# tdhock/PeakSegDisk

Hardware: AMD Instinct MI355X
Metric: coverage bins/sec across 64-penalty grid (higher is better)
Workload: dtype f64; 1 GPU; 1000000-bin synthetic Poisson coverage x 64-penalty grid per GPU (BASELINE.json configs[1]); bins=1000000, penalties=64, penalty_grid=10^seq(-1,5), 15 significant digits, seed=1+rank

## Files before the change

include/peaksegdisk_hip.h:

```cpp
#ifndef PEAKSEGDISK_HIP_H
#define PEAKSEGDISK_HIP_H

#include <stddef.h>

#ifdef __cplusplus
extern "C" {
#endif

#define ERROR_PENALTY_NOT_FINITE 1
#define ERROR_PENALTY_NEGATIVE 2
#define ERROR_UNABLE_TO_OPEN_BEDGRAPH 3
#define ERROR_NOT_ENOUGH_COLUMNS 4
#define ERROR_NON_INTEGER_DATA 5
#define ERROR_INCONSISTENT_CHROMSTART_CHROMEND 6
#define ERROR_WRITING_COST_FUNCTIONS 7
#define ERROR_WRITING_LOSS_OUTPUT 8
#define ERROR_NO_DATA 9
#define ERROR_PENALTY_NOT_NUMERIC 10
#define ERROR_WRITING_SEGMENTS_OUTPUT 11
#define ERROR_NO_HIP_DEVICE 12
#define ERROR_DEVICE_SOLVER 13
#define ERROR_DEVICE_MEMORY 14
#define ERROR_SEARCH_ARGUMENTS 15
#define ERROR_SEARCH_TOO_MANY_PEAKS 16
// ... 236 lines not shown
                                               const long long *contig_n_bases,
                                               const int *const *contig_counts, int counts_on_device,
                                               int n_penalties, const double *penalties,
                                               unsigned long long arena_pieces, int folds,
                                               unsigned long long seed, psd_problem_set **out);
int peakseg_hip_problem_set_create_reads_folds(
    int device, int n_contigs, const long long *n_reads, const int *const *read_start,
    const int *const *read_end, const int *const *read_count, int reads_on_device,
    const int *extent_start, const int *extent_end, int bases_counted, int n_penalties,
    const double *penalties, unsigned long long arena_pieces, int folds, unsigned long long seed,
    psd_problem_set **out);
int peakseg_hip_fold_max_count(void);
int peakseg_hip_fold_units_last_ms(float *ms);

int peakseg_hip_penalty_fit(int device, int n, int p, const double *x_std, const double *lo,
                            const double *hi, const int *fold, int n_folds, int n_reg,
                            const double *reg, double gram_lambda_max, double threshold,
                            int max_iterations, double *weights_out, int *iterations_out,
                            double *criterion_out, int *converged_out, long long *incorrect_out,
                            double *hinge_out);
int peakseg_hip_penalty_fit_last_ms(float *ms);
int peakseg_hip_penalty_fit_max_features(void);

int peakseg_hip_search_place_penalties(double under_penalty, double over_penalty, double secant,
                                       int extras, double *out);

int peakseg_hip_problem_set_loss(psd_problem_set *set, int problem, double *out);

long long peakseg_hip_problem_set_cycles(psd_problem_set *set, int problem);
void peakseg_hip_measured_rates(double *lat_rate, double *thr_rate);

long long peakseg_hip_spin_limit(void);
int peakseg_hip_problem_set_max_spin(psd_problem_set *set, int problem);

int peakseg_hip_problem_set_set_penalty(psd_problem_set *set, int problem, double penalty);

void peakseg_hip_problem_set_destroy(psd_problem_set *set);

int peakseg_hip_parse_probe(const char *path, int use_fast, int *n_lines,
                            unsigned long long *hash);

int peakseg_hip_dense_encode_probe(int device, int n_contigs, const long long *n_bases,
                                   const int *const *counts, int counts_on_device,
                                   long long *runs_out, int *count_out, int *weight_out,
                                   int *run_end_out, int *min_out, int *max_out,
                                   long long *sum_out);
int peakseg_hip_dense_tile_bases(void);
int peakseg_hip_dense_last_encode_ms(float *count_ms, float *scan_ms, float *scatter_ms);

int peakseg_hip_reads_pileup_probe(int device, int n_contigs, const long long *n_reads,
                                   const int *const *read_start, const int *const *read_end,
                                   const int *const *read_count, int reads_on_device,
                                   const int *extent_start, const int *extent_end, int bases_counted,
                                   int *coverage_out, long long *runs_out, int *count_out,
                                   int *weight_out, int *run_end_out);
int peakseg_hip_reads_last_pileup_ms(float *scatter_ms, float *scan_ms);

long long peakseg_hip_peak_clusters_probe(int device, int n_members, const long long *n_peaks,
                                          const int *const *peak_start, const int *const *peak_end,
                                          int *clusterStart_out, int *clusterEnd_out, int *peaks_out,
                                          int *samples_out, int *m_peaks_out);

int peakseg_hip_paste_double(double x, char *buf, size_t buf_len);

int peakseg_hip_problem_set_profile(psd_problem_set *set, int problem, long long *out);

// ... 10 lines not shown
```

peaksegdisk_amd/_native.py:

```python
import ctypes
import os

_HERE = os.path.dirname(os.path.abspath(__file__))
LIB_PATH = os.path.join(_HERE, "lib", "libpeaksegdisk_hip.so")

ERROR_NO_HIP_DEVICE = 12
ERROR_DEVICE_SOLVER = 13
ERROR_DEVICE_MEMORY = 14
ERROR_DENSE_ARGUMENTS = 17
ERROR_READS_ARGUMENTS = 18
ERROR_LABEL_ARGUMENTS = 19
ERROR_FEATURE_ARGUMENTS = 20
ERROR_FIT_ARGUMENTS = 21
ERROR_REGION_ARGUMENTS = 22
ERROR_HELDOUT_ARGUMENTS = 23


class PsdResult(ctypes.Structure):
    _fields_ = [
        ("status", ctypes.c_int),
        ("kernel_status", ctypes.c_int),
        ("n_segments", ctypes.c_int),
        ("n_peaks", ctypes.c_int),
        ("n_equality_constraints", ctypes.c_int),
# ... 93 lines not shown
    lib.PeakSegFPOP_parallel_search_batch.argtypes = [
        c.c_int, c.POINTER(c.c_char_p), c.POINTER(c.c_int), c.c_int, c.c_int, c.c_int,
        c.POINTER(PsdSearchRow), c.POINTER(c.c_int), c.POINTER(c.c_int), c.POINTER(c.c_int)]
    lib.PeakSegFPOP_parallel_search_batch.restype = c.c_int
    lib.peakseg_hip_problem_set_set_penalty.argtypes = [c.c_void_p, c.c_int, c.c_double]
    lib.peakseg_hip_problem_set_set_penalty.restype = c.c_int
    lib.peakseg_hip_problem_set_arena_bytes_used.argtypes = [c.c_void_p]
    lib.peakseg_hip_problem_set_arena_bytes_used.restype = c.c_ulonglong
    lib.peakseg_hip_problem_set_checkpoint_interval.argtypes = [c.c_void_p]
    lib.peakseg_hip_problem_set_checkpoint_interval.restype = c.c_int
    lib.peakseg_hip_paste_double.argtypes = [c.c_double, c.c_char_p, c.c_size_t]
    lib.peakseg_hip_paste_double.restype = c.c_int
    lib.peakseg_hip_problem_set_solve_stats.argtypes = [
        c.c_void_p, c.POINTER(c.c_int), c.POINTER(c.c_ulonglong)]
    lib.peakseg_hip_problem_set_solve_stats.restype = c.c_int
    lib.peakseg_hip_device_clock_khz.argtypes = [c.c_int]
    lib.peakseg_hip_device_clock_khz.restype = c.c_int
    lib.peakseg_hip_problem_set_park_stats.argtypes = [
        c.c_void_p, c.POINTER(c.c_int), c.POINTER(c.c_ulonglong)]
    lib.peakseg_hip_problem_set_park_stats.restype = c.c_int
    lib.peakseg_hip_problem_set_pack_tables.argtypes = [
        c.c_void_p, c.c_void_p, c.POINTER(c.c_void_p), c.POINTER(c.c_void_p)]
    lib.peakseg_hip_problem_set_pack_tables.restype = c.c_longlong
    lib.peakseg_hip_problem_set_packed_download.argtypes = [c.c_void_p, c.c_void_p, c.c_void_p]
    lib.peakseg_hip_problem_set_packed_download.restype = c.c_int
    lib.peakseg_hip_problem_set_cycles.argtypes = [c.c_void_p, c.c_int]
    lib.peakseg_hip_problem_set_cycles.restype = c.c_longlong
    lib.peakseg_hip_measured_rates.argtypes = [c.POINTER(c.c_double), c.POINTER(c.c_double)]
    lib.peakseg_hip_measured_rates.restype = None
    lib.peakseg_hip_spin_limit.argtypes = []
    lib.peakseg_hip_spin_limit.restype = c.c_longlong
    lib.peakseg_hip_problem_set_max_spin.argtypes = [c.c_void_p, c.c_int]
    lib.peakseg_hip_problem_set_max_spin.restype = c.c_int
    lib.peakseg_hip_last_warning.argtypes = []
    lib.peakseg_hip_last_warning.restype = c.c_char_p
    lib.peakseg_hip_problem_set_arena_stats.argtypes = [
        c.c_void_p, c.POINTER(c.c_ulonglong), c.POINTER(c.c_int), c.POINTER(c.c_int)]
    lib.peakseg_hip_problem_set_arena_stats.restype = c.c_int
    lib.peakseg_hip_last_fanout.argtypes = [
        c.c_int, c.POINTER(c.c_int), c.POINTER(c.c_int), c.POINTER(c.c_double)]
    lib.peakseg_hip_last_fanout.restype = c.c_int
    lib.peakseg_hip_last_fanout_entries.argtypes = [c.c_int, c.POINTER(c.c_int)]
    lib.peakseg_hip_last_fanout_entries.restype = c.c_int
    lib.peakseg_hip_problem_set_create_dense.argtypes = [
        c.c_int, c.c_int, c.POINTER(c.c_longlong), c.POINTER(c.c_void_p), c.c_int,
        c.c_int, c.POINTER(c.c_int), c.POINTER(c.c_double), c.c_ulonglong,
        c.POINTER(c.c_void_p)]
    lib.peakseg_hip_problem_set_create_dense.restype = c.c_int
    lib.peakseg_hip_problem_set_pack_segments.argtypes = [
        c.c_void_p, c.c_void_p, c.c_void_p, c.POINTER(c.c_void_p), c.POINTER(c.c_void_p),
        c.POINTER(c.c_void_p)]
    lib.peakseg_hip_problem_set_pack_segments.restype = c.c_longlong
    lib.peakseg_hip_problem_set_packed_segments_download.argtypes = [
        c.c_void_p, c.c_void_p, c.c_void_p, c.c_void_p]
    lib.peakseg_hip_problem_set_packed_segments_download.restype = c.c_int
    lib.peakseg_hip_problem_set_loss.argtypes = [c.c_void_p, c.c_int, c.POINTER(c.c_double)]
    lib.peakseg_hip_problem_set_loss.restype = c.c_int
    lib.peakseg_hip_dense_encode_probe.argtypes = [
        c.c_int, c.c_int, c.POINTER(c.c_longlong), c.POINTER(c.c_void_p), c.c_int,
        c.c_void_p, c.c_void_p, c.c_void_p, c.c_void_p, c.c_void_p, c.c_void_p, c.c_void_p]
    lib.peakseg_hip_dense_encode_probe.restype = c.c_int
    lib.peakseg_hip_dense_tile_bases.argtypes = []
    lib.peakseg_hip_dense_tile_bases.restype = c.c_int
    lib.peakseg_hip_dense_last_encode_ms.argtypes = [
        c.POINTER(c.c_float), c.POINTER(c.c_float), c.POINTER(c.c_float)]
    lib.peakseg_hip_dense_last_encode_ms.restype = c.c_int
# ... 117 lines not shown
        c.POINTER(c.c_double), c.c_ulonglong, c.c_int, c.c_ulonglong, c.POINTER(c.c_void_p)]
    lib.peakseg_hip_problem_set_create_dense_folds.restype = c.c_int
    lib.peakseg_hip_problem_set_create_reads_folds.argtypes = reads + [
        c.c_int, c.POINTER(c.c_double), c.c_ulonglong, c.c_int, c.c_ulonglong, c.POINTER(c.c_void_p)]
    lib.peakseg_hip_problem_set_create_reads_folds.restype = c.c_int
    lib.peakseg_hip_fold_max_count.argtypes = []
    lib.peakseg_hip_fold_max_count.restype = c.c_int
    lib.peakseg_hip_fold_units_last_ms.argtypes = [c.POINTER(c.c_float)]
    lib.peakseg_hip_fold_units_last_ms.restype = c.c_int
    lib.peakseg_hip_search_place_penalties.argtypes = [
        c.c_double, c.c_double, c.c_double, c.c_int, c.POINTER(c.c_double)]
    lib.peakseg_hip_search_place_penalties.restype = c.c_int
    return lib


EXPORTED_SYMBOLS = [
    "PeakSegFPOP_disk", "PeakSegFPOP_disk_batch", "PeakSegFPOP_status_message",
    "peakseg_hip_set_print", "peakseg_hip_device_count", "peakseg_hip_last_error",
    "peakseg_hip_problem_set_create", "peakseg_hip_problem_set_solve",
    "peakseg_hip_problem_set_result", "peakseg_hip_problem_set_segments",
    "peakseg_hip_problem_set_export_db", "peakseg_hip_problem_set_bytes",
    "peakseg_hip_problem_set_destroy", "peakseg_hip_math_probe", "peakseg_hip_parse_probe",
    "peakseg_hip_math_forms_probe",
    "peakseg_hip_problem_set_profile", "peakseg_hip_problem_set_kernel_build",
    "PeakSegFPOP_dir_batch", "PeakSegFPOP_sequential_search",
    "PeakSegFPOP_sequential_search_batch",
    "peakseg_hip_problem_set_set_penalty", "peakseg_hip_problem_set_arena_bytes_used",
    "peakseg_hip_paste_double", "peakseg_hip_problem_set_checkpoint_interval",
    "peakseg_hip_problem_set_solve_stats", "peakseg_hip_device_clock_khz",
    "peakseg_hip_last_warning", "peakseg_hip_problem_set_arena_stats",
    "peakseg_hip_problem_set_park_stats", "peakseg_hip_problem_set_pack_tables",
    "peakseg_hip_problem_set_packed_download", "peakseg_hip_problem_set_cycles",
    "peakseg_hip_measured_rates", "peakseg_hip_spin_limit", "peakseg_hip_problem_set_max_spin",
    "peakseg_hip_last_fanout", "peakseg_hip_last_fanout_entries",
    "PeakSegFPOP_parallel_search", "PeakSegFPOP_parallel_search_batch",
    "peakseg_hip_problem_set_create_dense", "peakseg_hip_problem_set_pack_segments",
    "peakseg_hip_problem_set_packed_segments_download", "peakseg_hip_problem_set_loss",
    "peakseg_hip_dense_encode_probe", "peakseg_hip_dense_tile_bases",
    "peakseg_hip_dense_last_encode_ms",
    "peakseg_hip_problem_set_pack_segment_stats",
    "peakseg_hip_problem_set_packed_segment_stats_download",
    "peakseg_hip_segment_stats_tile_runs", "peakseg_hip_segment_stats_last_ms",
    "peakseg_hip_problem_set_create_reads", "peakseg_hip_reads_pileup_probe",
    "peakseg_hip_reads_last_pileup_ms",
    "peakseg_hip_problem_set_pack_label_errors",
    "peakseg_hip_problem_set_packed_label_errors_download",
    "peakseg_hip_label_errors_last_ms", "peakseg_hip_search_place_penalties",
    "peakseg_hip_problem_set_pack_coverage_stats",
    "peakseg_hip_problem_set_packed_coverage_stats_download",
    "peakseg_hip_coverage_stats_tile_runs", "peakseg_hip_coverage_stats_max_ranks",
    "peakseg_hip_coverage_stats_last_ms", "peakseg_hip_coverage_stats_last_passes",
    "peakseg_hip_penalty_fit", "peakseg_hip_penalty_fit_last_ms",
    "peakseg_hip_penalty_fit_max_features",
    "peakseg_hip_problem_set_pack_region_stats",
    "peakseg_hip_problem_set_packed_region_stats_download",
    "peakseg_hip_region_stats_tile_runs", "peakseg_hip_region_stats_last_ms",
    "peakseg_hip_region_stats_last_fold_grid",
    "peakseg_hip_problem_set_pack_peak_clusters",
    "peakseg_hip_problem_set_packed_peak_clusters_download",
    "peakseg_hip_peak_clusters_last_ms", "peakseg_hip_peak_clusters_probe",
    "peakseg_hip_problem_set_pack_joint_peaks",
    "peakseg_hip_problem_set_packed_joint_peaks_download", "peakseg_hip_joint_peaks_last_ms",
    "peakseg_hip_joint_path_max_penalties", "peakseg_hip_problem_set_pack_joint_path",
    "peakseg_hip_problem_set_packed_joint_path_download", "peakseg_hip_joint_path_last_ms",
    "peakseg_hip_problem_set_pack_joint_label_errors",
    "peakseg_hip_problem_set_packed_joint_label_errors_download",
# ... 40 lines not shown
```

peaksegdisk_amd/csrc/fpop_kernels.h:

```cpp
#include "fpop_wave.h"
#include "fpop_arena.h"
#include "fpop_step.h"
#include "fpop_sync.h"
#include "fpop_ckpt.h"

#if defined(__clang__)
#pragma clang fp contract(off)
#endif

namespace psd {
namespace PSD_VARIANT {

struct BtState {
  double best_log_mean, prev_log_mean;
  int prev_seg_end, prev_seg_offset;
  int n_seg, n_eq, status;
};

PSD_D void backtrack_wave(const DeviceArgs &a, int p, int N, BtState &bt, unsigned long long fn_up,
                          unsigned long long fn_down, int t_origin, int t_lo) {
  const int lane = lane_id();
  int *seg_start = a.seg_start + a.prob_seg_off[p];
  double *seg_mean = a.seg_mean + a.prob_seg_off[p];
  double best_log_mean = bt.best_log_mean;
// ... 35 lines not shown
        prv = rec.prv[k];
        hit = mnk <= best_log_mean && best_log_mean <= mxk;
      }
      unsigned long long m = ballot(hit);
      if (m) {
        int src = ctz64(m);
        prev_seg_end = rdlane_i(di, src);
        prev_log_mean = rdlane_d(prv, src);
        found = true;
        break;
      }
    }
    if (!found) {
      status = PST_BACKTRACK;
      break;
    }
  }
  if (status == 0 && prev_seg_end < 0) {
    if (lane == 0) {
      seg_start[n_seg] = -1;
      seg_mean[n_seg] = d_exp(best_log_mean);
    }
    n_seg++;
  }
  bt.best_log_mean = best_log_mean;
  bt.prev_log_mean = prev_log_mean;
  bt.prev_seg_end = prev_seg_end;
  bt.prev_seg_offset = prev_seg_offset;
  bt.n_seg = n_seg;
  bt.n_eq = n_eq;
  bt.status = status;
}

#undef PSD_KERNEL_OCC
#if defined(PSD_KERNEL_WAVES_PER_EU) && !defined(PSD_EMU)
#define PSD_KERNEL_OCC \
  __attribute__((amdgpu_waves_per_eu(PSD_KERNEL_WAVES_PER_EU, PSD_KERNEL_WAVES_PER_EU)))
#else
#define PSD_KERNEL_OCC
#endif
template <bool CKPT>
PSD_D void forward_body(const DeviceArgs &a) {
  const int p = a.prob_order[blockIdx.x];
  const int chain = uniform_i(wave_id()) & 1;
  const int lane = lane_id();
  const int contig = a.prob_contig[p];
  const int N = a.contig_n[contig];
  const double penalty = a.prob_penalty[p];
  const int *count = a.count + a.contig_off[contig];
  const int *weight = a.weight + a.contig_off[contig];
  const LdsList mlist = lds_list(4 + chain);
  LdsScratch lsc;
  lsc.w = chain;

  psd_tables_init();
  if (threadIdx.x == 0) {
    if (a.started) atomicAdd_system(a.started, 1);
    g_sm.abort_status[0] = g_sm.abort_status[1] = g_sm.abort_status[2] = 0;
    g_sm.abort_err[0] = g_sm.abort_err[1] = g_sm.abort_err[2] = 0;
    for (int i = 0; i < 6; i++) g_sm.n[i] = 0;
    g_sm.serial[0] = g_sm.serial[1] = 0;
    g_sm.total_up = 0;
    g_sm.max_up = 0;
    g_sm.arrived[0] = g_sm.arrived[1] = 0xffffffffu;
#ifdef PSD_SPIN_STATS
    g_sm.spin_max[0] = g_sm.spin_max[1] = g_sm.spin_max[2] = g_sm.spin_max[3] = 0;
#endif
#ifdef PSD_PROFILE
    for (int i = 0; i < N_PROF; i++)
      g_sm.prof[0][i] = g_sm.prof[1][i] = g_sm.prof[2][i] = g_sm.prof[3][i] = 0;
#endif
#ifdef PSD_HELPER_WAVES
    for (int c = 0; c < 2; c++) {
      g_sm.mail[c].seq_cmd = g_sm.mail[c].seq_done = 0;
      g_sm.mail[c].op = 0;
      g_sm.mail[c].abort = 0;
    }
#endif
  }
  __syncthreads();
#ifdef PSD_HELPER_WAVES
  if (wave_id() >= 2) {
    helper_loop(chain, a);
    return;
  }
#endif

  const int K = CKPT ? a.ckpt_interval : 0;
  const unsigned long long fn_stride = K > 0 ? (unsigned long long)K + 1ull : (unsigned long long)N;
  const unsigned long long fn_up = (unsigned long long)a.prob_fn_off[p];
  const unsigned long long fn_down = fn_up + fn_stride;
  const unsigned long long fn_mine = chain == 1 ? fn_down : fn_up;
  ArenaCursor cur;
  cursor_clear(cur, K > 0 ? 0 : 1);
  unsigned long long total_intervals = 0;
  int max_intervals = 0;
  int spill_steps = 0;
  int status = 0;
  double cum_weight_i = 0.0, cum_weight_prev_i = -1.0;
  int cnt_reg = 0, wt_reg = 0;
  int b = 0;
  bool in_hbm = false;
  int spill_slot = -1;
  int t = 0;
  int t_lo = 0, t_hi = N;
  int t_first = 0;
  int t_origin = 0;
  int next_ckpt = K > 0 ? K : -1;
  bool forward = true;
  int step_reached = 0;
  int parked = 0;
  BtState bt;
  bt.best_log_mean = bt.prev_log_mean = 0.0;
  bt.prev_seg_end = -1;
  bt.prev_seg_offset = 0;
  bt.n_seg = bt.n_eq = bt.status = 0;
  ProbResult r;
  r.best_cost = 0.0;
  r.best_log_mean = 0.0;
  r.prev_log_mean = 0.0;
  r.prev_seg_end = -1;
  unsigned sync_no = 0;
  if (lane == 0) g_sm.t_begin[chain] = cycle_now();
  bool resumed_abort = false;
  if (!CKPT && a.prob_resume != nullptr) {
    const int t_resume = uniform_i(a.prob_resume[p]);
    if (t_resume > 0) {
      device_fence();
      in_hbm = uniform_i(ckpt_count(*a.self, p, 0, 0)) > LDS_CAP ||
               uniform_i(ckpt_count(*a.self, p, 0, 1)) > LDS_CAP;
      if (in_hbm) {
        spill_slot = uniform_i(take_spill_slot(*a.self, chain));
        if (spill_slot < 0) {
          status = PST_SPILL_FULL;
          resumed_abort = true;
          parked = 1;
          step_reached = t_resume;
        }
      }
      if (!resumed_abort) {
        const int n_ck = uniform_i(ckpt_load(*a.self, p, 0, chain, 2 * chain, in_hbm ? 1 : 0,
                                             spill_slot));
        if (lane == 0) g_sm.n[2 * chain] = n_ck;
        cum_weight_i = uniform_d(ckpt_cum_weight(*a.self, p, 0));
        cum_weight_prev_i = cum_weight_i;
        total_intervals = park_total_intervals(*a.self, p, chain);
        max_intervals = park_int(*a.self, p, 3 + chain);
        spill_steps = park_int(*a.self, p, 5);
        {
          const int n_serial = park_int(*a.self, p, 6 + chain);
          if (lane == 0) g_sm.serial[chain] = n_serial;
        }
        t_first = t_resume;
        block_sync(chain);
      }
    }
  }
  for (;;) {
  if (resumed_abort) break;
  for (t = t_first; t < t_hi; t++) {
    PSD_PROF_T0();
    if (!CKPT) cur.store = 1;
    if ((t & 63) == 0 || t == t_first) {
      int tt = (t & ~63) + lane;
      cnt_reg = tt < N ? count[tt] : 0;
      wt_reg = tt < N ? weight[tt] : 0;
    }
    const int coverage = rdlane_i(cnt_reg, t & 63);
    const double w = (double)rdlane_i(wt_reg, t & 63);
    const double cum_weight_new = cum_weight_i + w;
    const int nb = b ^ 1;
    const int id_own_prev = 2 * chain + b, id_own_new = 2 * chain + nb;
    const int id_other_prev = 2 * (1 - chain) + b;
    const int n_own = uniform_i(g_sm.n[id_own_prev]);
    const int n_other = uniform_i(g_sm.n[id_other_prev]);
    const unsigned long long fn_index = fn_mine + (unsigned long long)(t - t_origin);
    if (in_hbm && n_own <= LDS_CAP / 2 && n_other <= LDS_CAP / 2) {
      move_list_hbm(*a.self, spill_slot, id_own_prev, n_own, 0);
      in_hbm = false;
      block_sync(chain);
    }
    int n_new = 0;
    for (;;) {
      if (t == 0) {
        ArenaCursor cur0 = cur;
        n_new = uniform_i(first_point(*a.self, cur0, fn_index, chain, contig, coverage, id_own_new));
        cur = cur0;
      } else if (!in_hbm) {
#ifdef PSD_CALL_LDS_OPS
        n_new = chain_step<USE_HELPER>(a, cur, fn_index, chain, t,
                           lds_list(id_other_prev), n_other, lds_list(id_own_prev),
                           n_own, lds_list(id_own_new), mlist, lsc,
                           penalty / cum_weight_prev_i, cum_weight_prev_i, w, coverage,
                           cum_weight_new);
#else
        n_new = -WERR_SERIAL;
        if (t >= 2 && n_other <= FAST_MAX_OTHER && n_own <= FAST_MAX_OWN) {
          n_new = chain_step_fast<USE_HELPER>(
              a, cur, fn_index, chain, t, lds_list(id_other_prev), n_other,
              lds_list(id_own_prev), n_own, lds_list(id_own_new), mlist, lsc,
              penalty / cum_weight_prev_i, cum_weight_prev_i, w, coverage, cum_weight_new);
        }
        if (n_new == -WERR_SERIAL) {
          ArenaCursor cur_gen = cur;
          n_new = uniform_i(chain_step_lds<USE_HELPER>(
              *a.self, cur_gen, fn_index, chain, t, id_other_prev, n_other,
              id_own_prev, n_own, id_own_new, penalty / cum_weight_prev_i, cum_weight_prev_i, w,
              coverage, cum_weight_new));
          cur = cur_gen;
        }
#endif
      } else {
        ArenaCursor cur_hbm = cur;
        n_new = uniform_i(chain_step_hbm(*a.self, cur_hbm, fn_index, spill_slot, chain, t,
                               id_other_prev, n_other, id_own_prev, n_own, id_own_new,
                               penalty / cum_weight_prev_i, cum_weight_prev_i, w, coverage,
                               cum_weight_new));
        cur = cur_hbm;
        block_sync_cold(chain);
      }
      PSD_PROF_T0();
      const unsigned slot = sync_no % 3u;
      if (lane == 0) g_sm.n[id_own_new] = n_new < 0 ? 0 : n_new;
      if (n_new < 0) {
        if (lane == 0) {
          g_sm.abort_err[slot] = -n_new;
          g_sm.abort_status[slot] = ((-n_new) & WERR_ARENA)      ? PST_ARENA_FULL
                                    : ((-n_new) & WERR_OVERFLOW) ? PST_LDS_OVERFLOW
                                                                 : PST_REF_THROW;
        }
      }
      PSD_PROF_ADD(PROF_ARENA);
      if (!step_sync(chain, sync_no)) {
        status = PST_REF_THROW;
        if (lane == 0) g_sm.abort_err[slot] = WERR_HELPER;
        break;
      }
      PSD_PROF_ADD(PROF_BARRIER);
      status = uniform_i(g_sm.abort_status[slot]);
      if (lane == 0) g_sm.abort_status[(sync_no + 2u) % 3u] = 0;
      sync_no++;
#ifdef PSD_PARK_ON_LDS_OVERFLOW
      if (status == PST_LDS_OVERFLOW && !CKPT && a.prob_resume != nullptr && t > 0) break;
#endif
      if (status == PST_LDS_OVERFLOW && !in_hbm && a.spill_cap > LDS_CAP && t > 0) {
        if (spill_slot < 0) {
          spill_slot = uniform_i(take_spill_slot(*a.self, chain));
          if (spill_slot < 0) {
            status = PST_SPILL_FULL;
            break;
          }
        }
        move_list_hbm(*a.self, spill_slot, id_own_prev, n_own, 1);
        in_hbm = true;
        status = 0;
        block_sync(chain);
        continue;
      }
      break;
    }
    if (status != 0) {
#ifdef PSD_PARK_ON_LDS_OVERFLOW
      const bool park_now = status == PST_ARENA_FULL || status == PST_SPILL_FULL ||
                            status == PST_LDS_OVERFLOW;
#else
      const bool park_now = status == PST_ARENA_FULL || status == PST_SPILL_FULL;
#endif
      if (!CKPT && park_now && a.prob_resume != nullptr && t > 0) {
        const int n_up = uniform_i(g_sm.n[b]), n_down = uniform_i(g_sm.n[2 + b]);
        unsigned long long ovf = 0;
        bool can_park = true;
        if (n_up > a.ckpt_cap || n_down > a.ckpt_cap) {
          ovf = psd_d2u(uniform_d(psd_u2d(ckpt_take_overflow(*a.self, chain, n_up, n_down))));
          if (ovf == ~0ull) can_park = false;
          if (can_park && chain == 1 && n_up > a.ckpt_cap) ovf += (unsigned long long)n_up;
        }
        if (can_park) {
          ckpt_save(*a.self, p, 0, chain, 2 * chain + b, chain == 0 ? n_up : n_down, cum_weight_i,
                    in_hbm ? 1 : 0, spill_slot, ovf);
          park_counters_save(*a.self, p, chain, t, total_intervals, max_intervals, spill_steps);
          parked = 1;
        }
      }
      break;
    }
    if (!CKPT || forward) {
      total_intervals += (unsigned long long)n_new;
      if (max_intervals < n_new) max_intervals = n_new;
      if (in_hbm) spill_steps++;
    }
    cum_weight_i = cum_weight_new;
    cum_weight_prev_i = cum_weight_i;
    b = nb;
    if (CKPT && t == next_ckpt) {
      const int n_up = uniform_i(g_sm.n[b]), n_down = uniform_i(g_sm.n[2 + b]);
      unsigned long long ovf = 0;
      if (n_up > a.ckpt_cap || n_down > a.ckpt_cap) {
        ovf = psd_d2u(uniform_d(psd_u2d(ckpt_take_overflow(*a.self, chain, n_up, n_down))));
        if (ovf == ~0ull) {
          status = PST_CKPT_FULL;
          break;
        }
        if (chain == 1 && n_up > a.ckpt_cap) ovf += (unsigned long long)n_up;
      }
      ckpt_save(*a.self, p, t / K - 1, chain, 2 * chain + b, n_new, cum_weight_i, in_hbm ? 1 : 0,
                spill_slot, ovf);
      next_ckpt += K;
    }
  }
  if (!CKPT || forward) step_reached = t;
  if (status != 0) break;
  if (forward) {
    if (chain == 0 && lane == 0) {
      g_sm.total_up = total_intervals;
      g_sm.max_up = max_intervals;
    }
  }
  device_fence();
  block_sync(chain);
  if (chain == 1) {
    if (forward) {
      const int id = 2 + b;
      if (in_hbm) {
        minimize_wave(global_list(a, spill_slot, id), g_sm.n[id], &r.best_cost, &r.best_log_mean,
                      &r.prev_seg_end, &r.prev_log_mean);
      } else {
        minimize_wave(lds_list(id), g_sm.n[id], &r.best_cost, &r.best_log_mean, &r.prev_seg_end,
                      &r.prev_log_mean);
      }
      bt.best_log_mean = r.best_log_mean;
      bt.prev_log_mean = r.prev_log_mean;
      bt.prev_seg_end = r.prev_seg_end;
    }
    backtrack_wave(a, p, N, bt, fn_up, fn_down, t_origin, (K > 0 && forward) ? N : t_lo);
  }
  if (!CKPT || K == 0) break;
  if (chain == 1 && lane == 0) {
    int c = -1;
    if (bt.status == 0 && bt.prev_seg_end >= 0)
      c = bt.prev_seg_end == 0 ? 0 : (bt.prev_seg_end - 1) / K;
    g_sm.bt_next = c;
  }
  block_sync(chain);
  const int c = uniform_i(g_sm.bt_next);
  if (c < 0) break;
  forward = false;
  next_ckpt = -1;
  t_origin = c * K;
  t_lo = c == 0 ? 0 : c * K + 1;
  t_hi = (c + 1) * K + 1 < N ? (c + 1) * K + 1 : N;
  t_first = t_lo;
  {
    const unsigned long long per_block = (1ull << a.ar_block_log2) / a.ckpt_region;
    const unsigned long long region = (unsigned long long)p * 2ull + (unsigned long long)chain;
    cursor_point(a, cur, ((region / per_block) << a.ar_block_log2) + (region % per_block) * a.ckpt_region,
                 (int)a.ckpt_region);
    cur.store = 1;
  }
  in_hbm = false;
  b = 0;
  if (c == 0) {
    cum_weight_i = 0.0;
    cum_weight_prev_i = -1.0;
    if (lane == 0) g_sm.n[2 * chain] = g_sm.n[2 * chain + 1] = 0;
  } else {
    device_fence();
    in_hbm = uniform_i(ckpt_count(*a.self, p, c - 1, 0)) > LDS_CAP ||
             uniform_i(ckpt_count(*a.self, p, c - 1, 1)) > LDS_CAP;
    if (in_hbm && spill_slot < 0) {
      spill_slot = uniform_i(take_spill_slot(*a.self, chain));
      if (spill_slot < 0) {
        status = PST_SPILL_FULL;
        break;
      }
    }
    const int n_ck = uniform_i(ckpt_load(*a.self, p, c - 1, chain, 2 * chain, in_hbm ? 1 : 0,
                                         spill_slot));
    if (lane == 0) g_sm.n[2 * chain] = n_ck;
    cum_weight_i = uniform_d(ckpt_cum_weight(*a.self, p, c - 1));
    cum_weight_prev_i = cum_weight_i;
  }
  block_sync(chain);
  }
#ifdef PSD_HELPER_WAVES
  if (mail_wait(chain)) mail_post(chain, HOP_EXIT);
  else if (lane == 0) g_sm.mail[chain].abort = 1;
#endif
#ifdef PSD_PROFILE
  if (lane == 0 && a.prof) {
    long long *dst = a.prof + ((long long)p * 2 + chain) * N_PROF;
    for (int i = 0; i < N_PROF; i++) dst[i] = g_sm.prof[chain][i];
    dst[PROF_TOTAL] = cycle_now() - g_sm.t_begin[chain];
  }
#endif
  if (chain == 1) {
    r.status = status != 0 ? status : bt.status;
    r.wave_err = g_sm.abort_err[0] | g_sm.abort_err[1] | g_sm.abort_err[2];
    r.max_intervals = max_intervals > g_sm.max_up ? max_intervals : g_sm.max_up;
    r.total_intervals = total_intervals + g_sm.total_up;
    r.n_segments = bt.n_seg;
    r.n_equality = bt.n_eq;
    r.n_serial_env = g_sm.serial[0] + g_sm.serial[1];
    r.step_reached = step_reached;
    r.spill_steps = spill_steps;
    r.parked = parked;
    r.max_spin = 0;
#ifdef PSD_SPIN_STATS
    for (int w = 0; w < 4; w++) r.max_spin = g_sm.spin_max[w] > r.max_spin ? g_sm.spin_max[w] : r.max_spin;
#endif
    r.cycles = cycle_now() - g_sm.t_begin[chain];
    if (lane == 0) a.result[p] = r;
  }
}

__global__ __launch_bounds__(FORWARD_THREADS) PSD_KERNEL_OCC void fpop_forward_kernel(
    DeviceArgs a) {
  forward_body<false>(a);
}
__global__ __launch_bounds__(FORWARD_THREADS) PSD_KERNEL_OCC void fpop_forward_ckpt_kernel(
    DeviceArgs a) {
  forward_body<true>(a);
}

__global__ void math_probe_kernel(int op, int n, const double *x, double *y) {
  psd_tables_init();
  int i = (int)(blockIdx.x * blockDim.x + threadIdx.x);
  if (i < n) {
    if (op == 2)
      y[i] = psd_div(x[i], x[n + i]);
    else if (op == 3)
      y[i] = x[i] / x[n + i];
    else
      y[i] = op == 0 ? d_exp(x[i]) : d_log(x[i]);
  }
}

}
}
```

peaksegdisk_amd/csrc/fpop_lds.h:

```cpp
#if defined(__clang__)
#pragma clang fp contract(off)
#endif

namespace psd {
namespace PSD_VARIANT {

constexpr int LDS_CAP = PSD_LDS_CAP;

struct ListStore {
  double Lin[LDS_CAP], Log[LDS_CAP], Con[LDS_CAP], mn[LDS_CAP], mx[LDS_CAP], prv[LDS_CAP];
  int di[LDS_CAP];
};
struct ScratchStore {
  double lc[LDS_CAP], rc[LDS_CAP];
  double om[LDS_CAP], mu[LDS_CAP];
  double muc[LDS_CAP], oc2[LDS_CAP];
  int cls[LDS_CAP];
  int iv[2 * LDS_CAP];
};
enum {
  HOP_BARRIER = 1, HOP_EXIT = 2, HOP_ROOT = 3,
  HOP_HBM_COSTS = 4,
  HOP_HBM_TABLE = 5,
  HOP_HBM_CLASSIFY = 6,
};
struct Mail {
  int seq_cmd, seq_done, op, abort;
  int h_arg[8];
  int h_progress;
  int flags[64];
  double d_lin[64], d_log[64], d_con[64], b[64];
  double res_large[64];
};

struct SharedBlock {
  ListStore list[6];
  ScratchStore sc[2];
  unsigned arrived[2];
  int n[6];
  int abort_status[3];
  int abort_err[3];
  unsigned long long total_up;
  int max_up;
  int serial[2];
  int spill_slot;
  int bt_next;
  unsigned long long ckpt_ovf;
#ifdef PSD_HELPER_WAVES
  Mail mail[2];
#endif
#ifdef PSD_PROFILE
  long long prof[4][N_PROF];
#endif
#ifdef PSD_SPIN_STATS
  int spin_max[4];
#endif
  long long t_begin[2];
  unsigned long long cur_ptr[2][3];
};

PSD_LDS SharedBlock g_sm;

constexpr int WAIT_SPIN_LIMIT = 1 << 26;
#ifdef PSD_SPIN_STATS
#define PSD_SPIN_NOTE(spin)                                                           \
  do {                                                                                \
    if (lane_id() == 0 && (spin) > g_sm.spin_max[wave_id()]) g_sm.spin_max[wave_id()] = (spin); \
  } while (0)
#else
#define PSD_SPIN_NOTE(spin) \
  do {                      \
  } while (0)
#endif
#ifdef PSD_HELPER_WAVES
constexpr int MAIL_SPIN_LIMIT = WAIT_SPIN_LIMIT;
PSD_D bool mail_wait(int chain) {
  Mail &m = g_sm.mail[chain];
  const int want = flag_load(&m.seq_cmd);
  for (int spin = 0; spin < MAIL_SPIN_LIMIT; spin++) {
    if (flag_load(&m.seq_done) == want) {
      PSD_SPIN_NOTE(spin);
      return true;
    }
    spin_pause();
  }
  return false;
}
PSD_D void mail_post(int chain, int op) {
// ... 221 lines not shown
```

peaksegdisk_amd/csrc/fpop_types.h:

```cpp
#ifndef PSD_FPOP_TYPES_H
#define PSD_FPOP_TYPES_H

namespace psd {

constexpr int N_PROF = 24;

constexpr int ARENA_CHUNK_LOG2_MAX = 16;
constexpr int ARENA_CHUNK_LOG2_MIN = 10;
constexpr int ARENA_BLOCK_LOG2_MIN = 19;
constexpr int ARENA_BLOCK_LOG2_MAX = 24;
constexpr int ARENA_BLOCK_LOG2_CKPT_MAX = 30;
constexpr int FN_COUNT_BITS = 24;
constexpr int SPILL_CAP_MAX = 32767;

enum {
  PST_OK = 0,
  PST_LDS_OVERFLOW = 1,
  PST_ARENA_FULL = 2,
  PST_REF_THROW = 3,
  PST_BACKTRACK = 4,
  PST_SPILL_FULL = 5,
  PST_CKPT_SPILL = 6,
  PST_CKPT_FULL = 7,
};

struct ProbResult {
  double best_cost;
  double best_log_mean;
  double prev_log_mean;
  int prev_seg_end;
  int status;
  int wave_err;
  int max_intervals;
  unsigned long long total_intervals;
  int n_segments;
  int n_equality;
  int n_serial_env;
  int step_reached;
  int spill_steps;
  int parked;
  int max_spin;
  long long cycles;
};

struct DeviceArgs {
  const DeviceArgs *self;
  int n_problems;
  const int *prob_contig;
  const double *prob_penalty;
  const long long *prob_fn_off;
  const long long *prob_seg_off;
  const int *prob_order;
  ProbResult *result;
  const int *contig_n;
  const long long *contig_off;
  const double *contig_min_log_mean;
  const double *contig_max_log_mean;
  const int *count;
  const int *weight;
  char **ar_block;
  int ar_block_log2;
  unsigned long long ar_cap;
  const unsigned long long *ar_live;
  unsigned long long *ar_used;
  const int *prob_resume;
  int ar_chunk_log2;
  unsigned long long *ar_next_chunk;
  unsigned long long *fn_ref;
  int *seg_start;
  double *seg_mean;
  long long *prof;
  double *spill_f64;
  int *spill_i32;
  int spill_cap;
// ... 18 lines not shown
```

peaksegdisk_amd/csrc/peakseg_hip.cpp:

```cpp
#include "../../include/peaksegdisk_hip.h"

#define PSD_VARIANT lat
#define PSD_LDS_CAP 128
#define PSD_MATH_VK 1
#define PSD_HELPER_WAVES 1
#define PSD_FLAG_BARRIER 1
#include "fpop_kernels.h"
#undef PSD_VARIANT
#undef PSD_LDS_CAP
#undef PSD_HELPER_WAVES
#undef PSD_FLAG_BARRIER
#undef PSD_MATH_VK
#define PSD_VARIANT thr
#ifndef PSD_THR_LDS_CAP
#define PSD_THR_LDS_CAP 64
#endif
#ifndef PSD_THR_WAVES_PER_EU
#define PSD_THR_WAVES_PER_EU 2
#endif
#define PSD_LDS_CAP PSD_THR_LDS_CAP
#define PSD_KERNEL_WAVES_PER_EU PSD_THR_WAVES_PER_EU
#define PSD_CALL_LDS_OPS 1
#include "fpop_kernels.h"
#undef PSD_VARIANT
// ... 389 lines not shown
  double *out[3] = {y0, y1, lz};
  for (int k = 0; k < 3; k++)
    if (out[k]) HIP_TRY(hipMemcpy(out[k], d[3 + k], bytes, hipMemcpyDeviceToHost));
  if (rare) HIP_TRY(hipMemcpy(rare, d_rare, (size_t)n * 4, hipMemcpyDeviceToHost));
  for (auto &q : d) (void)hipFree(q);
  (void)hipFree(d_rare);
  return 0;
}

extern "C" int peakseg_hip_problem_set_park_stats(psd_problem_set *s, int *parks,
                                                  unsigned long long *overflow_pool_pieces) {
  if (!s) return -1;
  if (parks) *parks = s->run.parks;
  if (overflow_pool_pieces) *overflow_pool_pieces = s->run.park_pool_pieces;
  return 0;
}

extern "C" long long peakseg_hip_problem_set_cycles(psd_problem_set *s, int p) {
  if (!s || !s->solved || p < 0 || p >= s->n_problems) return -1;
  return s->results[(size_t)p].cycles;
}

extern "C" void peakseg_hip_measured_rates(double *lat_rate, double *thr_rate) {
  if (lat_rate) *lat_rate = g_lat_rate.load();
  if (thr_rate) *thr_rate = g_thr_rate.load();
}

extern "C" long long peakseg_hip_spin_limit(void) { return (long long)psd::lat::WAIT_SPIN_LIMIT; }
extern "C" int peakseg_hip_problem_set_max_spin(psd_problem_set *s, int p) {
  if (!s || !s->solved || p < 0 || p >= s->n_problems) return -1;
  return s->results[(size_t)p].max_spin;
}

#include "peakseg_fanout.h"
#include "peakseg_files.h"
#include "peakseg_dir.h"
#include "peakseg_search.h"

extern "C" char *PeakSegFPOP_status_message(int status, const char *bedGraph, const char *penalty,
                                            const char *db, char *buf, size_t buf_len) {
  if (!buf || buf_len == 0) return buf;
  buf[0] = 0;
#define PSD_MESSAGE(code, ...) case code: snprintf(buf, buf_len, __VA_ARGS__); break
  switch (status) {
    case 0:
      break;
    PSD_MESSAGE(ERROR_PENALTY_NOT_FINITE, "penalty=%s but must be finite", penalty);
    PSD_MESSAGE(ERROR_PENALTY_NEGATIVE, "penalty=%s must be non-negative", penalty);
    PSD_MESSAGE(ERROR_UNABLE_TO_OPEN_BEDGRAPH, "unable to open input file for reading %s", bedGraph);
    PSD_MESSAGE(ERROR_NOT_ENOUGH_COLUMNS,
                "each line of input data file %s should have exactly four columns", bedGraph);
    PSD_MESSAGE(ERROR_NON_INTEGER_DATA, "fourth column of input data file %s should be integer",
                bedGraph);
    PSD_MESSAGE(ERROR_INCONSISTENT_CHROMSTART_CHROMEND,
                "there should be no gaps (columns 2-3) in input data file %s", bedGraph);
    PSD_MESSAGE(ERROR_WRITING_COST_FUNCTIONS, "unable to write to cost function database file %s", db);
    PSD_MESSAGE(ERROR_WRITING_LOSS_OUTPUT, "unable to write to loss output file %s_penalty=%s_loss.tsv",
                bedGraph, penalty);
    PSD_MESSAGE(ERROR_WRITING_SEGMENTS_OUTPUT,
                "unable to write to segments output file %s_penalty=%s_segments.bed", bedGraph, penalty);
    PSD_MESSAGE(ERROR_NO_DATA, "input file %s contains no data", bedGraph);
    PSD_MESSAGE(ERROR_PENALTY_NOT_NUMERIC,
                "penalty string '%s' is not numeric; it should be convertible to double", penalty);
    PSD_MESSAGE(ERROR_NO_HIP_DEVICE,
                "error code %d: no HIP device (MI355X) is visible and this solver has no CPU path", status);
    PSD_MESSAGE(ERROR_DENSE_ARGUMENTS,
// ... 38 lines not shown
```

peaksegdisk_amd/csrc/psd_platform.h:

```cpp
#ifndef PSD_PLATFORM_H
#define PSD_PLATFORM_H

#ifdef PSD_EMU
#include "hip_emu.h"
#include <time.h>
#define PSD_D static inline
#define PSD_M inline
#define PSD_NOINLINE static __attribute__((noinline))
#define PSD_LDS static thread_local
#define PSD_COLD_DEV static __attribute__((noinline, cold))
#else
#include <hip/hip_runtime.h>
#define PSD_D __device__ __forceinline__
#define PSD_M __device__ __forceinline__
#define PSD_NOINLINE __device__ __attribute__((noinline))
#define PSD_LDS __shared__
#define PSD_COLD_DEV __device__ __attribute__((noinline, cold))
#endif

#ifdef PSD_EMU
typedef double gdouble;
typedef int gint;
typedef unsigned long long gull;
typedef double ldouble;
// ... 121 lines not shown
PSD_D void atomic_max_u64(unsigned long long *p, unsigned long long v) {
  unsigned long long o = __atomic_load_n(p, __ATOMIC_RELAXED);
  while (v > o && !__atomic_compare_exchange_n(p, &o, v, false, __ATOMIC_RELAXED, __ATOMIC_RELAXED)) {
  }
}
PSD_D void atomic_max_i32(int *p, int v) {
  int o = __atomic_load_n(p, __ATOMIC_RELAXED);
  while (v > o && !__atomic_compare_exchange_n(p, &o, v, false, __ATOMIC_RELAXED, __ATOMIC_RELAXED)) {
  }
}
#else
PSD_D void atomic_add_i32(int *p, int v) {
  (void)__hip_atomic_fetch_add(p, v, __ATOMIC_RELAXED, __HIP_MEMORY_SCOPE_AGENT);
}
PSD_D void atomic_add_i64(long long *p, long long v) {
  (void)__hip_atomic_fetch_add(p, v, __ATOMIC_RELAXED, __HIP_MEMORY_SCOPE_AGENT);
}
PSD_D void atomic_max_u64(unsigned long long *p, unsigned long long v) {
  (void)__hip_atomic_fetch_max(p, v, __ATOMIC_RELAXED, __HIP_MEMORY_SCOPE_AGENT);
}
PSD_D void atomic_max_i32(int *p, int v) {
  (void)__hip_atomic_fetch_max(p, v, __ATOMIC_RELAXED, __HIP_MEMORY_SCOPE_AGENT);
}
#endif

#ifdef PSD_EMU
PSD_D void lds_add_u32(unsigned *p, unsigned v) { *p += v; }
#else
PSD_D void lds_add_u32(unsigned *p, unsigned v) {
  (void)__hip_atomic_fetch_add(p, v, __ATOMIC_RELAXED, __HIP_MEMORY_SCOPE_WORKGROUP);
}
#endif

template <class T>
PSD_D T *uniform_p(T *p) {
#ifdef PSD_EMU
  return p;
#else
  uint64_t u = (uint64_t)p;
  uint32_t lo = (uint32_t)__builtin_amdgcn_readfirstlane((int)(uint32_t)u);
  uint32_t hi = (uint32_t)__builtin_amdgcn_readfirstlane((int)(uint32_t)(u >> 32));
  return (T *)(((uint64_t)hi << 32) | lo);
#endif
}

#ifdef PSD_EMU
PSD_D unsigned long long mul_wide_u64(unsigned long long a, unsigned long long b,
                                      unsigned long long &hi) {
  const unsigned __int128 p = (unsigned __int128)a * b;
  hi = (unsigned long long)(p >> 64);
  return (unsigned long long)p;
}
#else
PSD_D unsigned long long mul_wide_u64(unsigned long long a, unsigned long long b,
                                      unsigned long long &hi) {
  hi = __umul64hi(a, b);
  return a * b;
}
#endif

PSD_D int popc64(unsigned long long m) { return __builtin_popcountll(m); }
PSD_D int ctz64(unsigned long long m) { return __builtin_ctzll(m); }
PSD_D int msb64(unsigned long long m) { return 63 - __builtin_clzll(m); }
PSD_D unsigned long long lanes_below(int lane) { return (1ull << lane) - 1ull; }

}
#endif
```

Measured before the change: 6.457 million bins/s.

## Add a tight fast-path inner loop for non-checkpoint LDS steps

For the non-checkpoint forward pass with lists resident in LDS, the step loop gains a dedicated inner loop. It calls chain_step_fast directly, publishes results, syncs the two chains, and advances t without going through the general loop's branching, spill checks and bookkeeping. Scalar kernel arguments are made wave-uniform with readfirstlane so they can sit in scalar registers. The running interval counters are pinned to vector registers so they do not spill. Optional loop-count statistics are added behind a compile flag. The cost is more code and a more complex control flow, and the break-out into the general path depends on the synced and reload flags being handled correctly.

After: 6.683 million bins/s (median of 6 runs). +3.5%, better.

```diff
diff --git a/include/peaksegdisk_hip.h b/include/peaksegdisk_hip.h
--- a/include/peaksegdisk_hip.h
+++ b/include/peaksegdisk_hip.h
@@ -292,6 +292,7 @@
 
 long long peakseg_hip_spin_limit(void);
 int peakseg_hip_problem_set_max_spin(psd_problem_set *set, int problem);
+int peakseg_hip_problem_set_loop_stats(psd_problem_set *set, int problem, int *out);
 
 int peakseg_hip_problem_set_set_penalty(psd_problem_set *set, int problem, double penalty);
 
diff --git a/peaksegdisk_amd/_native.py b/peaksegdisk_amd/_native.py
--- a/peaksegdisk_amd/_native.py
+++ b/peaksegdisk_amd/_native.py
@@ -149,6 +149,8 @@
     lib.peakseg_hip_spin_limit.restype = c.c_longlong
     lib.peakseg_hip_problem_set_max_spin.argtypes = [c.c_void_p, c.c_int]
     lib.peakseg_hip_problem_set_max_spin.restype = c.c_int
+    lib.peakseg_hip_problem_set_loop_stats.argtypes = [c.c_void_p, c.c_int, c.POINTER(c.c_int)]
+    lib.peakseg_hip_problem_set_loop_stats.restype = c.c_int
     lib.peakseg_hip_last_warning.argtypes = []
     lib.peakseg_hip_last_warning.restype = c.c_char_p
     lib.peakseg_hip_problem_set_arena_stats.argtypes = [
@@ -332,6 +334,7 @@
     "peakseg_hip_problem_set_park_stats", "peakseg_hip_problem_set_pack_tables",
     "peakseg_hip_problem_set_packed_download", "peakseg_hip_problem_set_cycles",
     "peakseg_hip_measured_rates", "peakseg_hip_spin_limit", "peakseg_hip_problem_set_max_spin",
+    "peakseg_hip_problem_set_loop_stats",
     "peakseg_hip_last_fanout", "peakseg_hip_last_fanout_entries",
     "PeakSegFPOP_parallel_search", "PeakSegFPOP_parallel_search_batch",
     "peakseg_hip_problem_set_create_dense", "peakseg_hip_problem_set_pack_segments",
diff --git a/peaksegdisk_amd/csrc/fpop_kernels.h b/peaksegdisk_amd/csrc/fpop_kernels.h
--- a/peaksegdisk_amd/csrc/fpop_kernels.h
+++ b/peaksegdisk_amd/csrc/fpop_kernels.h
@@ -91,6 +91,31 @@
   bt.status = status;
 }
 
+PSD_D void step_publish(int lane, int id_own_new, int n_new, unsigned slot) {
+  if (lane == 0) g_sm.n[id_own_new] = n_new < 0 ? 0 : n_new;
+  if (n_new < 0) {
+    if (lane == 0) {
+      g_sm.abort_err[slot] = -n_new;
+      g_sm.abort_status[slot] = ((-n_new) & WERR_ARENA)      ? PST_ARENA_FULL
+                                : ((-n_new) & WERR_OVERFLOW) ? PST_LDS_OVERFLOW
+                                                             : PST_REF_THROW;
+    }
+  }
+}
+
+enum { LOOP_INSIDE = 0, LOOP_GENERAL = 1, LOOP_ENTRIES = 2 };
+#undef PSD_LOOP_COUNT
+#ifdef PSD_LOOP_STATS
+#define PSD_LOOP_COUNT(which)                                   \
+  do {                                                          \
+    if (lane_id() == 0) g_sm.loop_stats[wave_id() & 1][which]++; \
+  } while (0)
+#else
+#define PSD_LOOP_COUNT(which) \
+  do {                        \
+  } while (0)
+#endif
+
 #undef PSD_KERNEL_OCC
 #if defined(PSD_KERNEL_WAVES_PER_EU) && !defined(PSD_EMU)
 #define PSD_KERNEL_OCC \
@@ -100,14 +125,15 @@
 #endif
 template <bool CKPT>
 PSD_D void forward_body(const DeviceArgs &a) {
-  const int p = a.prob_order[blockIdx.x];
+  const int p = uniform_i(a.prob_order[blockIdx.x]);
   const int chain = uniform_i(wave_id()) & 1;
   const int lane = lane_id();
-  const int contig = a.prob_contig[p];
-  const int N = a.contig_n[contig];
-  const double penalty = a.prob_penalty[p];
-  const int *count = a.count + a.contig_off[contig];
-  const int *weight = a.weight + a.contig_off[contig];
+  const int contig = uniform_i(a.prob_contig[p]);
+  const int N = uniform_i(a.contig_n[contig]);
+  const double penalty = uniform_d(a.prob_penalty[p]);
+  const long long contig_off = (long long)uniform_u64((unsigned long long)a.contig_off[contig]);
+  const int *count = a.count + contig_off;
+  const int *weight = a.weight + contig_off;
   const LdsList mlist = lds_list(4 + chain);
   LdsScratch lsc;
   lsc.w = chain;
@@ -125,6 +151,9 @@
 #ifdef PSD_SPIN_STATS
     g_sm.spin_max[0] = g_sm.spin_max[1] = g_sm.spin_max[2] = g_sm.spin_max[3] = 0;
 #endif
+#ifdef PSD_LOOP_STATS
+    for (int i = 0; i < 3; i++) g_sm.loop_stats[0][i] = g_sm.loop_stats[1][i] = 0;
+#endif
 #ifdef PSD_PROFILE
     for (int i = 0; i < N_PROF; i++)
       g_sm.prof[0][i] = g_sm.prof[1][i] = g_sm.prof[2][i] = g_sm.prof[3][i] = 0;
@@ -147,7 +176,7 @@
 
   const int K = CKPT ? a.ckpt_interval : 0;
   const unsigned long long fn_stride = K > 0 ? (unsigned long long)K + 1ull : (unsigned long long)N;
-  const unsigned long long fn_up = (unsigned long long)a.prob_fn_off[p];
+  const unsigned long long fn_up = uniform_u64((unsigned long long)a.prob_fn_off[p]);
   const unsigned long long fn_down = fn_up + fn_stride;
   const unsigned long long fn_mine = chain == 1 ? fn_down : fn_up;
   ArenaCursor cur;
@@ -159,14 +188,14 @@
   double cum_weight_i = 0.0, cum_weight_prev_i = -1.0;
   int cnt_reg = 0, wt_reg = 0;
   int b = 0;
-  bool in_hbm = false;
+  int in_hbm = 0;
   int spill_slot = -1;
   int t = 0;
   int t_lo = 0, t_hi = N;
   int t_first = 0;
   int t_origin = 0;
   int next_ckpt = K > 0 ? K : -1;
-  bool forward = true;
+  int forward = 1;
   int step_reached = 0;
   int parked = 0;
   BtState bt;
@@ -181,18 +210,18 @@
   r.prev_seg_end = -1;
   unsigned sync_no = 0;
   if (lane == 0) g_sm.t_begin[chain] = cycle_now();
-  bool resumed_abort = false;
+  int resumed_abort = 0;
   if (!CKPT && a.prob_resume != nullptr) {
     const int t_resume = uniform_i(a.prob_resume[p]);
     if (t_resume > 0) {
       device_fence();
-      in_hbm = uniform_i(ckpt_count(*a.self, p, 0, 0)) > LDS_CAP ||
-               uniform_i(ckpt_count(*a.self, p, 0, 1)) > LDS_CAP;
+      in_hbm = (uniform_i(ckpt_count(*a.self, p, 0, 0)) > LDS_CAP ||
+                uniform_i(ckpt_count(*a.self, p, 0, 1)) > LDS_CAP) ? 1 : 0;
       if (in_hbm) {
         spill_slot = uniform_i(take_spill_slot(*a.self, chain));
         if (spill_slot < 0) {
           status = PST_SPILL_FULL;
-          resumed_abort = true;
+          resumed_abort = 1;
           parked = 1;
           step_reached = t_resume;
         }
@@ -203,9 +232,9 @@
         if (lane == 0) g_sm.n[2 * chain] = n_ck;
         cum_weight_i = uniform_d(ckpt_cum_weight(*a.self, p, 0));
         cum_weight_prev_i = cum_weight_i;
-        total_intervals = park_total_intervals(*a.self, p, chain);
-        max_intervals = park_int(*a.self, p, 3 + chain);
-        spill_steps = park_int(*a.self, p, 5);
+        total_intervals = uniform_u64(park_total_intervals(*a.self, p, chain));
+        max_intervals = uniform_i(park_int(*a.self, p, 3 + chain));
+        spill_steps = uniform_i(park_int(*a.self, p, 5));
         {
           const int n_serial = park_int(*a.self, p, 6 + chain);
           if (lane == 0) g_sm.serial[chain] = n_serial;
@@ -217,13 +246,81 @@
   }
   for (;;) {
   if (resumed_abort) break;
+  int reload = 1;
   for (t = t_first; t < t_hi; t++) {
+    int synced = 0;
+#ifndef PSD_CALL_LDS_OPS
+    if (!CKPT && t >= 2 && !in_hbm) {
+      int entry = 1;
+      cur.store = 1;
+      unsigned long long total_v = total_intervals;
+      int max_v = max_intervals;
+      PSD_VECTOR_REG(total_v);
+      PSD_VECTOR_REG(max_v);
+      for (;;) {
+        PSD_PROF_T0();
+        const int nb = b ^ 1;
+        const int n_own = uniform_i(g_sm.n[2 * chain + b]);
+        const int n_other = uniform_i(g_sm.n[2 * (1 - chain) + b]);
+        if (n_other > FAST_MAX_OTHER || n_own > FAST_MAX_OWN) break;
+        if (entry || (t & 63) == 0) {
+          int tt = (t & ~63) + lane;
+          cnt_reg = tt < N ? count[tt] : 0;
+          wt_reg = tt < N ? weight[tt] : 0;
+          if (entry) PSD_LOOP_COUNT(LOOP_ENTRIES);
+          entry = 0;
+        }
+        const int coverage = rdlane_i(cnt_reg, t & 63);
+        const double w = (double)rdlane_i(wt_reg, t & 63);
+        const double cum_weight_new = cum_weight_i + w;
+        double pen_term = 0.0;
+        if (chain == 0) pen_term = penalty / cum_weight_prev_i;
+        const int n_new = uniform_i(chain_step_fast<USE_HELPER>(
+            a, cur, fn_mine + (unsigned long long)(t - t_origin), chain, t,
+            lds_list(2 * (1 - chain) + b), n_other, lds_list(2 * chain + b), n_own,
+            lds_list(2 * chain + nb), mlist, lsc, pen_term, cum_weight_prev_i, w, coverage,
+            cum_weight_new));
+        if (n_new == -WERR_SERIAL) break;
+        synced = 1;
+        {
+          PSD_PROF_T0();
+          const unsigned slot = sync_no % 3u;
+          step_publish(lane, 2 * chain + nb, n_new, slot);
+          PSD_PROF_ADD(PROF_ARENA);
+          if (!step_sync(chain, sync_no)) {
+            status = PST_REF_THROW;
+            if (lane == 0) g_sm.abort_err[slot] = WERR_HELPER;
+            break;
+          }
+          PSD_PROF_ADD(PROF_BARRIER);
+          status = uniform_i(g_sm.abort_status[slot]);
+          if (lane == 0) g_sm.abort_status[(sync_no + 2u) % 3u] = 0;
+          sync_no++;
+        }
+        if (status != 0) break;
+        synced = 0;
+        PSD_LOOP_COUNT(LOOP_INSIDE);
+        total_v += (unsigned long long)n_new;
+        if (max_v < n_new) max_v = n_new;
+        cum_weight_i = cum_weight_new;
+        cum_weight_prev_i = cum_weight_i;
+        b = nb;
+        t++;
+        if (t >= t_hi) break;
+      }
+      total_intervals = uniform_u64(total_v);
+      max_intervals = uniform_i(max_v);
+      if (!entry) reload = 1;
+      if (t >= t_hi) break;
+    }
+#endif
     PSD_PROF_T0();
     if (!CKPT) cur.store = 1;
-    if ((t & 63) == 0 || t == t_first) {
+    if ((t & 63) == 0 || reload) {
       int tt = (t & ~63) + lane;
       cnt_reg = tt < N ? count[tt] : 0;
       wt_reg = tt < N ? weight[tt] : 0;
+      reload = 0;
     }
     const int coverage = rdlane_i(cnt_reg, t & 63);
     const double w = (double)rdlane_i(wt_reg, t & 63);
@@ -236,11 +333,12 @@
     const unsigned long long fn_index = fn_mine + (unsigned long long)(t - t_origin);
     if (in_hbm && n_own <= LDS_CAP / 2 && n_other <= LDS_CAP / 2) {
       move_list_hbm(*a.self, spill_slot, id_own_prev, n_own, 0);
-      in_hbm = false;
+      in_hbm = 0;
       block_sync(chain);
     }
     int n_new = 0;
     for (;;) {
+      if (!synced) {
       if (t == 0) {
         ArenaCursor cur0 = cur;
         n_new = uniform_i(first_point(*a.self, cur0, fn_index, chain, contig, coverage, id_own_new));
@@ -254,11 +352,11 @@
                            cum_weight_new);
 #else
         n_new = -WERR_SERIAL;
-        if (t >= 2 && n_other <= FAST_MAX_OTHER && n_own <= FAST_MAX_OWN) {
-          n_new = chain_step_fast<USE_HELPER>(
+        if (CKPT && t >= 2 && n_other <= FAST_MAX_OTHER && n_own <= FAST_MAX_OWN) {
+          n_new = uniform_i(chain_step_fast<USE_HELPER>(
               a, cur, fn_index, chain, t, lds_list(id_other_prev), n_other,
               lds_list(id_own_prev), n_own, lds_list(id_own_new), mlist, lsc,
-              penalty / cum_weight_prev_i, cum_weight_prev_i, w, coverage, cum_weight_new);
+              penalty / cum_weight_prev_i, cum_weight_prev_i, w, coverage, cum_weight_new));
         }
         if (n_new == -WERR_SERIAL) {
           ArenaCursor cur_gen = cur;
@@ -280,15 +378,7 @@
       }
       PSD_PROF_T0();
       const unsigned slot = sync_no % 3u;
-      if (lane == 0) g_sm.n[id_own_new] = n_new < 0 ? 0 : n_new;
-      if (n_new < 0) {
-        if (lane == 0) {
-          g_sm.abort_err[slot] = -n_new;
-          g_sm.abort_status[slot] = ((-n_new) & WERR_ARENA)      ? PST_ARENA_FULL
-                                    : ((-n_new) & WERR_OVERFLOW) ? PST_LDS_OVERFLOW
-                                                                 : PST_REF_THROW;
-        }
-      }
+      step_publish(lane, id_own_new, n_new, slot);
       PSD_PROF_ADD(PROF_ARENA);
       if (!step_sync(chain, sync_no)) {
         status = PST_REF_THROW;
@@ -299,6 +389,8 @@
       status = uniform_i(g_sm.abort_status[slot]);
       if (lane == 0) g_sm.abort_status[(sync_no + 2u) % 3u] = 0;
       sync_no++;
+      }
+      synced = 0;
 #ifdef PSD_PARK_ON_LDS_OVERFLOW
       if (status == PST_LDS_OVERFLOW && !CKPT && a.prob_resume != nullptr && t > 0) break;
 #endif
@@ -311,7 +403,7 @@
           }
         }
         move_list_hbm(*a.self, spill_slot, id_own_prev, n_own, 1);
-        in_hbm = true;
+        in_hbm = 1;
         status = 0;
         block_sync(chain);
         continue;
@@ -343,6 +435,7 @@
       }
       break;
     }
+    PSD_LOOP_COUNT(LOOP_GENERAL);
     if (!CKPT || forward) {
       total_intervals += (unsigned long long)n_new;
       if (max_intervals < n_new) max_intervals = n_new;
@@ -403,7 +496,7 @@
   block_sync(chain);
   const int c = uniform_i(g_sm.bt_next);
   if (c < 0) break;
-  forward = false;
+  forward = 0;
   next_ckpt = -1;
   t_origin = c * K;
   t_lo = c == 0 ? 0 : c * K + 1;
@@ -416,7 +509,7 @@
                  (int)a.ckpt_region);
     cur.store = 1;
   }
-  in_hbm = false;
+  in_hbm = 0;
   b = 0;
   if (c == 0) {
     cum_weight_i = 0.0;
@@ -424,8 +517,8 @@
     if (lane == 0) g_sm.n[2 * chain] = g_sm.n[2 * chain + 1] = 0;
   } else {
     device_fence();
-    in_hbm = uniform_i(ckpt_count(*a.self, p, c - 1, 0)) > LDS_CAP ||
-             uniform_i(ckpt_count(*a.self, p, c - 1, 1)) > LDS_CAP;
+    in_hbm = (uniform_i(ckpt_count(*a.self, p, c - 1, 0)) > LDS_CAP ||
+              uniform_i(ckpt_count(*a.self, p, c - 1, 1)) > LDS_CAP) ? 1 : 0;
     if (in_hbm && spill_slot < 0) {
       spill_slot = uniform_i(take_spill_slot(*a.self, chain));
       if (spill_slot < 0) {
@@ -467,6 +560,9 @@
 #ifdef PSD_SPIN_STATS
     for (int w = 0; w < 4; w++) r.max_spin = g_sm.spin_max[w] > r.max_spin ? g_sm.spin_max[w] : r.max_spin;
 #endif
+#ifdef PSD_LOOP_STATS
+    for (int i = 0; i < 6; i++) r.loop_stats[i] = g_sm.loop_stats[i / 3][i % 3];
+#endif
     r.cycles = cycle_now() - g_sm.t_begin[chain];
     if (lane == 0) a.result[p] = r;
   }
diff --git a/peaksegdisk_amd/csrc/fpop_lds.h b/peaksegdisk_amd/csrc/fpop_lds.h
--- a/peaksegdisk_amd/csrc/fpop_lds.h
+++ b/peaksegdisk_amd/csrc/fpop_lds.h
@@ -54,6 +54,9 @@
 #endif
 #ifdef PSD_SPIN_STATS
   int spin_max[4];
+#endif
+#ifdef PSD_LOOP_STATS
+  int loop_stats[2][3];
 #endif
   long long t_begin[2];
   unsigned long long cur_ptr[2][3];
diff --git a/peaksegdisk_amd/csrc/fpop_types.h b/peaksegdisk_amd/csrc/fpop_types.h
--- a/peaksegdisk_amd/csrc/fpop_types.h
+++ b/peaksegdisk_amd/csrc/fpop_types.h
@@ -40,6 +40,9 @@
   int spill_steps;
   int parked;
   int max_spin;
+#ifdef PSD_LOOP_STATS
+  int loop_stats[6];
+#endif
   long long cycles;
 };
 
diff --git a/peaksegdisk_amd/csrc/peakseg_hip.cpp b/peaksegdisk_amd/csrc/peakseg_hip.cpp
--- a/peaksegdisk_amd/csrc/peakseg_hip.cpp
+++ b/peaksegdisk_amd/csrc/peakseg_hip.cpp
@@ -445,6 +445,16 @@
   return s->results[(size_t)p].max_spin;
 }
 
+extern "C" int peakseg_hip_problem_set_loop_stats(psd_problem_set *s, int p, int *out) {
+  if (!s || !s->solved || p < 0 || p >= s->n_problems || !out) return -1;
+#ifdef PSD_LOOP_STATS
+  for (int i = 0; i < 6; i++) out[i] = s->results[(size_t)p].loop_stats[i];
+  return 6;
+#else
+  return 0;
+#endif
+}
+
 #include "peakseg_fanout.h"
 #include "peakseg_files.h"
 #include "peakseg_dir.h"
diff --git a/peaksegdisk_amd/csrc/psd_platform.h b/peaksegdisk_amd/csrc/psd_platform.h
--- a/peaksegdisk_amd/csrc/psd_platform.h
+++ b/peaksegdisk_amd/csrc/psd_platform.h
@@ -177,6 +177,14 @@
 }
 #endif
 
+#ifdef PSD_EMU
+#define PSD_VECTOR_REG(x) \
+  do {                    \
+  } while (0)
+#else
+#define PSD_VECTOR_REG(x) asm("" : "+v"(x))
+#endif
+
 template <class T>
 PSD_D T *uniform_p(T *p) {
 #ifdef PSD_EMU
@@ -186,6 +194,16 @@
   uint32_t lo = (uint32_t)__builtin_amdgcn_readfirstlane((int)(uint32_t)u);
   uint32_t hi = (uint32_t)__builtin_amdgcn_readfirstlane((int)(uint32_t)(u >> 32));
   return (T *)(((uint64_t)hi << 32) | lo);
+#endif
+}
+
+PSD_D unsigned long long uniform_u64(unsigned long long v) {
+#ifdef PSD_EMU
+  return v;
+#else
+  uint32_t lo = (uint32_t)__builtin_amdgcn_readfirstlane((int)(uint32_t)v);
+  uint32_t hi = (uint32_t)__builtin_amdgcn_readfirstlane((int)(uint32_t)(v >> 32));
+  return ((unsigned long long)hi << 32) | lo;
 #endif
 }
 
```
